# yuliakot/snark-verifier-axiom

Hardware: AMD Instinct MI355X
Metric: BN254 G1 MSM points/sec at 2^20 + KZG pairings/sec; 1/2/4/8 GPU (higher is better)
Workload: dtype u32 (254-bit Montgomery field: bucket chain 9x29-bit limbs, elsewhere 8x32-bit)

## Files before the change

### snark-verifier-axiom_amd/csrc/msm.hip

```cpp
#include <hip/hip_runtime.h>

#include <algorithm>
#include <chrono>
#include <cmath>
#include <cstdio>
#include <cstdlib>
#include <cstring>
#include <atomic>
#include <functional>
#include <string>
#include <thread>
#include <type_traits>
#include <vector>

#include "curve.hpp"
#include "curve29.hpp"
#include "glv.hpp"
#include "host_ec.hpp"
#include "msm.hpp"
#include "msm_batch.hpp"
#include "quad.hpp"
#include "runtime.hpp"

namespace sv {
// ... 144 lines not shown
    } else {
      f(w, bits, 0u);
      carry = 0;
    }
  }
}

__device__ __forceinline__ Fr scalar_in(const uint4 q0, const uint4 q1, int mont_in, uint32_t* __restrict__ err) {
  Fr s;
  s.v[0] = q0.x; s.v[1] = q0.y; s.v[2] = q0.z; s.v[3] = q0.w;
  s.v[4] = q1.x; s.v[5] = q1.y; s.v[6] = q1.z; s.v[7] = q1.w;
  if (err && !s.is_reduced()) atomicOr(err, 2u);
  return mont_in ? fe_from_mont(s) : s;
}
__device__ __forceinline__ Fr load_scalar(const Fr* __restrict__ scalars, uint32_t i, int mont_in,
                                          uint32_t* __restrict__ err) {
  const uint4* p = reinterpret_cast<const uint4*>(scalars + i);
  const uint4 q0 = p[0], q1 = p[1];
  Fr s;
  s.v[0] = q0.x; s.v[1] = q0.y; s.v[2] = q0.z; s.v[3] = q0.w;
  s.v[4] = q1.x; s.v[5] = q1.y; s.v[6] = q1.z; s.v[7] = q1.w;
  if (err && !s.is_reduced()) atomicOr(err, 2u);
  return mont_in ? fe_from_mont(s) : s;
}

template <int C, bool GLV>
struct Digits {
  static constexpr int NB = GLV ? 128 : 255;
  static constexpr int W = num_windows<C, NB>();
  static constexpr int EP = GLV ? 2 * W : W;
  uint32_t h[GLV ? 2 : 1][GLV ? 4 : 8];
  uint32_t sgn[GLV ? 2 : 1];
  __device__ __forceinline__ void load(const Fr* __restrict__ scalars, uint32_t i, int mont_in,
                                       uint32_t* __restrict__ err) {
    from(load_scalar(scalars, i, mont_in, err));
  }
  __device__ __forceinline__ void from(const Fr& s) {
    if constexpr (GLV) {
      uint32_t h1[4], h2[4];
      glv_split(s.v, h1, h2);
#pragma unroll
      for (int k = 0; k < 4; k++) h[0][k] = h1[k], h[1][k] = h2[k];
#pragma unroll
      for (int q = 0; q < 2; q++) {
        sgn[q] = h[q][3] >> 31;
        h[q][3] &= 0x7fffffffu;
      }
    } else {
#pragma unroll
      for (int k = 0; k < 8; k++) h[0][k] = s.v[k];
      sgn[0] = 0;
    }
  }
  __device__ __forceinline__ void store(uint4* __restrict__ hv, uint32_t i) const {
    if constexpr (GLV) {
      hv[2 * i] = make_uint4(h[0][0], h[0][1], h[0][2], h[0][3] | (sgn[0] << 31));
      hv[2 * i + 1] = make_uint4(h[1][0], h[1][1], h[1][2], h[1][3] | (sgn[1] << 31));
    } else {
      hv[2 * i] = make_uint4(h[0][0], h[0][1], h[0][2], h[0][3]);
      hv[2 * i + 1] = make_uint4(h[0][4], h[0][5], h[0][6], h[0][7]);
    }
  }
  __device__ __forceinline__ void load_stored(const uint4* __restrict__ hv, uint32_t i) {
    const uint4 a = hv[2 * i], b = hv[2 * i + 1];
    if constexpr (GLV) {
      h[0][0] = a.x; h[0][1] = a.y; h[0][2] = a.z; h[0][3] = a.w & 0x7fffffffu;
      h[1][0] = b.x; h[1][1] = b.y; h[1][2] = b.z; h[1][3] = b.w & 0x7fffffffu;
      sgn[0] = a.w >> 31;
      sgn[1] = b.w >> 31;
    } else {
      h[0][0] = a.x; h[0][1] = a.y; h[0][2] = a.z; h[0][3] = a.w;
      h[0][4] = b.x; h[0][5] = b.y; h[0][6] = b.z; h[0][7] = b.w;
      sgn[0] = 0;
    }
  }
  template <class F>
  __device__ __forceinline__ void each(F&& f) const {
#pragma unroll
    for (int q = 0; q < (GLV ? 2 : 1); q++) {
      Fr s;
      if constexpr (GLV) {
#pragma unroll
        for (int k = 0; k < 4; k++) s.v[k] = h[q][k], s.v[4 + k] = 0u;
      } else {
#pragma unroll
        for (int k = 0; k < 8; k++) s.v[k] = h[0][k];
      }
      const uint32_t sg = sgn[q];
      for_each_digit<C, NB>(s, [&](int w, uint32_t mag, uint32_t neg) { f(w, mag, neg ^ sg, (uint32_t)q); });
    }
  }
};

__device__ __forceinline__ void glv_phix(const G1Aff* __restrict__ bases, uint32_t i, uint4* __restrict__ phix,
                                         int phi64, uint32_t* __restrict__ err) {
  const uint4* b = reinterpret_cast<const uint4*>(bases + i);
  Fq x, beta;
  const uint4 x0 = b[0], x1 = b[1];
  x.v[0] = x0.x; x.v[1] = x0.y; x.v[2] = x0.z; x.v[3] = x0.w;
  x.v[4] = x1.x; x.v[5] = x1.y; x.v[6] = x1.z; x.v[7] = x1.w;
#pragma unroll
  for (int j = 0; j < 8; j++) beta.v[j] = GLV_BETA_MONT[j];
  const Fq bx = x * beta;
  uint4* o = phix + (phi64 ? 4 : 2) * i;
  o[0] = make_uint4(bx.v[0], bx.v[1], bx.v[2], bx.v[3]);
  o[1] = make_uint4(bx.v[4], bx.v[5], bx.v[6], bx.v[7]);
  if (phi64 || err) {
    const uint4 y0 = b[2], y1 = b[3];
    if (phi64) {
      o[2] = y0;
      o[3] = y1;
    }
    if (err) {
      Fq y;
      y.v[0] = y0.x; y.v[1] = y0.y; y.v[2] = y0.z; y.v[3] = y0.w;
      y.v[4] = y1.x; y.v[5] = y1.y; y.v[6] = y1.z; y.v[7] = y1.w;
      if (!x.is_reduced() || !y.is_reduced()) atomicOr(err, 1u);
    }
  }
}

__global__ void k_glv_phix(const G1Aff* __restrict__ bases, uint32_t n, uint4* __restrict__ phix, int phi64,
                           uint32_t* __restrict__ err) {
  const uint32_t i = blockIdx.x * blockDim.x + threadIdx.x;
  if (i < n) glv_phix(bases, i, phix, phi64, err);
}

static constexpr int kPhiVtab = 2;
static constexpr int kVtabRec = 9;
static constexpr uint32_t kVtabIdentity = 0x80000000u;
__device__ __forceinline__ void st_rec29(uint2* o, const r29::F& x, const r29::F& y) {
  o[0] = make_uint2(x.v[0], x.v[1]);
  o[1] = make_uint2(x.v[2], x.v[3]);
  o[2] = make_uint2(x.v[4], x.v[5]);
  o[3] = make_uint2(x.v[6], x.v[7]);
  o[4] = make_uint2(x.v[8], y.v[0]);
  o[5] = make_uint2(y.v[1], y.v[2]);
  o[6] = make_uint2(y.v[3], y.v[4]);
  o[7] = make_uint2(y.v[5], y.v[6]);
  o[8] = make_uint2(y.v[7], y.v[8]);
}
__device__ __forceinline__ void ld_rec29(const uint2* __restrict__ o, r29::F& x, r29::F& y) {
  uint2 q[kVtabRec];
#pragma unroll
  for (int k = 0; k < kVtabRec; k++) q[k] = o[k];
  x.v[0] = q[0].x, x.v[1] = q[0].y, x.v[2] = q[1].x, x.v[3] = q[1].y, x.v[4] = q[2].x, x.v[5] = q[2].y;
  x.v[6] = q[3].x, x.v[7] = q[3].y, x.v[8] = q[4].x;
  y.v[0] = q[4].y, y.v[1] = q[5].x, y.v[2] = q[5].y, y.v[3] = q[6].x, y.v[4] = q[6].y, y.v[5] = q[7].x;
  y.v[6] = q[7].y, y.v[7] = q[8].x, y.v[8] = q[8].y;
}
__device__ __forceinline__ void vtab_put_pt(const G1Aff& a, uint32_t i, uint4* __restrict__ vtab, uint32_t nsplit,
                                            bool glv, uint32_t* __restrict__ err) {
  if (err && (!a.x.is_reduced() || !a.y.is_reduced())) atomicOr(err, 1u);
  r29::F y = r29::to_r29(a.y.v);
  const r29::F x = r29::to_r29(a.x.v);
  if (r29::is_zero(x) && r29::is_zero(y)) y.v[r29::L - 1] = kVtabIdentity;
  uint2* t = reinterpret_cast<uint2*>(vtab);
  st_rec29(t + kVtabRec * (size_t)i, x, y);
  if (glv) {
    constexpr uint32_t kBeta29[r29::L] = {0xa337995u, 0x158d1d23u, 0x189c9b98u, 0x12fa4e45u, 0x185faadcu,
                                         0x176f16du, 0xeed93bau,  0x14291140u, 0xc0afeu};
    r29::F beta;
#pragma unroll
    for (int j = 0; j < r29::L; j++) beta.v[j] = kBeta29[j];
    st_rec29(t + kVtabRec * ((size_t)nsplit + i), r29::mul(x, beta), y);
  }
}
__device__ __forceinline__ void vtab_put(const G1Aff* __restrict__ bases, uint32_t i, uint4* __restrict__ vtab,
                                         uint32_t nsplit, bool glv, uint32_t* __restrict__ err) {
  vtab_put_pt(load_aff(bases, i), i, vtab, nsplit, glv, err);
}
__global__ void k_vtab(const G1Aff* __restrict__ bases, uint32_t n, uint4* __restrict__ vtab, int glv,
                       uint32_t* __restrict__ err) {
  const uint32_t i = blockIdx.x * blockDim.x + threadIdx.x;
  if (i < n) vtab_put(bases, i, vtab, n, glv != 0, err);
}

__global__ void __launch_bounds__(kBlock) k_resident_prepare(const G1Aff* in, G1Aff* out, uint32_t n, int mont_in,
                                                             uint4* __restrict__ vtab, uint32_t* __restrict__ err) {
  const uint32_t i = blockIdx.x * blockDim.x + threadIdx.x;
  if (i >= n) return;
  G1Aff a;
  {
    const uint4* p = reinterpret_cast<const uint4*>(in + i);
    const uint4 q0 = p[0], q1 = p[1], q2 = p[2], q3 = p[3];
    a.x.v[0] = q0.x; a.x.v[1] = q0.y; a.x.v[2] = q0.z; a.x.v[3] = q0.w;
    a.x.v[4] = q1.x; a.x.v[5] = q1.y; a.x.v[6] = q1.z; a.x.v[7] = q1.w;
    a.y.v[0] = q2.x; a.y.v[1] = q2.y; a.y.v[2] = q2.z; a.y.v[3] = q2.w;
    a.y.v[4] = q3.x; a.y.v[5] = q3.y; a.y.v[6] = q3.z; a.y.v[7] = q3.w;
  }
  if (!a.x.is_reduced() || !a.y.is_reduced()) {
    atomicOr(err, 1u);
    a.x = Fq::zero();
    a.y = Fq::zero();
  }
  if (!mont_in && !a.is_identity()) {
    a.x = fe_to_mont(a.x);
    a.y = fe_to_mont(a.y);
  }
  uint4* o = reinterpret_cast<uint4*>(out + i);
  o[0] = make_uint4(a.x.v[0], a.x.v[1], a.x.v[2], a.x.v[3]);
  o[1] = make_uint4(a.x.v[4], a.x.v[5], a.x.v[6], a.x.v[7]);
  o[2] = make_uint4(a.y.v[0], a.y.v[1], a.y.v[2], a.y.v[3]);
  o[3] = make_uint4(a.y.v[4], a.y.v[5], a.y.v[6], a.y.v[7]);
  vtab_put_pt(a, i, vtab, n, true, nullptr);
}

__global__ void k_check_bases(const G1Aff* __restrict__ bases, uint32_t n, uint32_t* __restrict__ err) {
  const uint32_t i = blockIdx.x * blockDim.x + threadIdx.x;
  if (i >= n) return;
  const G1Aff a = load_aff(bases, i);
  if (!a.x.is_reduced() || !a.y.is_reduced()) atomicOr(err, 1u);
}

__host__ __device__ constexpr int ceil_log2(int x) { return x <= 1 ? 0 : 1 + ceil_log2((x + 1) / 2); }

template <int N>
__device__ __forceinline__ uint32_t block_excl_scan(uint32_t* x, uint32_t* part) {
  constexpr int PER = (N + kBlock - 1) / kBlock;
  const int tid = threadIdx.x;
  uint32_t loc[PER];
  uint32_t sum = 0;
#pragma unroll
  for (int j = 0; j < PER; j++) {
    const int k = tid * PER + j;
    loc[j] = k < N ? x[k] : 0u;
    sum += loc[j];
  }
  part[tid] = sum;
  __syncthreads();
  for (int off = 1; off < kBlock; off <<= 1) {
    const uint32_t u = tid >= off ? part[tid - off] : 0u;
    __syncthreads();
    part[tid] += u;
    __syncthreads();
  }
  uint32_t run = part[tid] - sum;
  const uint32_t total = part[kBlock - 1];
#pragma unroll
  for (int j = 0; j < PER; j++) {
    const int k = tid * PER + j;
    if (k < N) x[k] = run;
    run += loc[j];
  }
  __syncthreads();
  return total;
}

__device__ __forceinline__ uint32_t pack_entry32(uint32_t fine, uint32_t neg, uint32_t pt, uint32_t fb) {
  return (fb ? fine << (32 - fb) : 0u) | (neg << (31 - fb)) | pt;
}
__device__ __forceinline__ uint64_t load_entry(const uint64_t* __restrict__ tmp, uint32_t i, int e32, uint32_t fb) {
  if (!e32) return tmp[i];
  const uint32_t v = reinterpret_cast<const uint32_t*>(tmp)[i];
  const uint32_t fine = fb ? v >> (32 - fb) : 0u, neg = (v >> (31 - fb)) & 1u, pt = v & ((1u << (31 - fb)) - 1u);
  return ((uint64_t)fine << 32) | pt | (neg << 31);
}

__device__ __forceinline__ uint32_t sort_block(uint32_t b, uint32_t n, int xcd) {
  const uint32_t nfull = n & ~7u;
  if (!xcd || b >= nfull) return b;
  return (b & 7u) * (nfull >> 3) + (b >> 3);
}

template <int C, bool GLV>
__global__ void __launch_bounds__(kBlock) k_bin_hist(const Fr* __restrict__ scalars, uint32_t n, int mont_in,
                                                     uint32_t nblk, uint32_t* __restrict__ bcnt,
                                                     uint32_t* __restrict__ err, const G1Aff* __restrict__ bases,
                                                     uint4* __restrict__ phix, int phi64, int check_bases,
                                                     int xcd, int bm, uint32_t w0, uint32_t nw,
                                                     uint4* __restrict__ stored, int pf) {
  using D = Digits<C, GLV>;
  constexpr int W = D::W, LOGB = C - 1;
  constexpr int CB = coarse_bits(C, D::NB), FB = LOGB - CB, NBIN = 1 << CB;
  const uint32_t nk = nw * NBIN;
  __shared__ uint32_t h[W * NBIN];
  for (int k = threadIdx.x; k < W * NBIN; k += kBlock) h[k] = 0;
  __syncthreads();
  constexpr uint32_t CH = sort_chunk(D::EP);
  const uint32_t blk = sort_block(blockIdx.x, gridDim.x, xcd);
  const uint32_t lo = blk * CH, hi = min(n, lo + CH);
  auto count = [&](const D& d) {
    d.each([&](int w, uint32_t mag, uint32_t, uint32_t) {
      if (mag && (uint32_t)w - w0 < nw) atomicAdd(&h[(w - w0) * NBIN + ((mag - 1) >> FB)], 1u);
    });
  };
  if (phix && phi64 == kPhiVtab && pf) {
    uint32_t i = lo + threadIdx.x;
    const uint4* sp = reinterpret_cast<const uint4*>(scalars);
    const uint4* bp = reinterpret_cast<const uint4*>(bases);
    uint4 s0{}, s1{}, b0{}, b1{}, b2{}, b3{};
    if (i < hi) {
      s0 = sp[2 * (size_t)i], s1 = sp[2 * (size_t)i + 1];
      b0 = bp[4 * (size_t)i], b1 = bp[4 * (size_t)i + 1], b2 = bp[4 * (size_t)i + 2], b3 = bp[4 * (size_t)i + 3];
    }
    for (; i < hi; i += kBlock) {
      G1Aff a;
      a.x.v[0] = b0.x; a.x.v[1] = b0.y; a.x.v[2] = b0.z; a.x.v[3] = b0.w;
      a.x.v[4] = b1.x; a.x.v[5] = b1.y; a.x.v[6] = b1.z; a.x.v[7] = b1.w;
      a.y.v[0] = b2.x; a.y.v[1] = b2.y; a.y.v[2] = b2.z; a.y.v[3] = b2.w;
      a.y.v[4] = b3.x; a.y.v[5] = b3.y; a.y.v[6] = b3.z; a.y.v[7] = b3.w;
      const uint4 c0 = s0, c1 = s1;
      const uint32_t j = i + kBlock;
      if (j < hi) {
        s0 = sp[2 * (size_t)j], s1 = sp[2 * (size_t)j + 1];
        b0 = bp[4 * (size_t)j], b1 = bp[4 * (size_t)j + 1], b2 = bp[4 * (size_t)j + 2], b3 = bp[4 * (size_t)j + 3];
      }
      vtab_put_pt(a, i, phix, n, GLV, check_bases ? err : nullptr);
      D d;
      d.from(scalar_in(c0, c1, mont_in, err));
      if (stored) d.store(stored, i);
      count(d);
    }
  } else
  for (uint32_t i = lo + threadIdx.x; i < hi; i += kBlock) {
    if (phix && phi64 == kPhiVtab) {
      vtab_put(bases, i, phix, n, GLV, check_bases ? err : nullptr);
    } else if constexpr (GLV) {
      if (phix) glv_phix(bases, i, phix, phi64, check_bases ? err : nullptr);
    } else {
      if (check_bases) {
        const G1Aff a = load_aff(bases, i);
        if (!a.x.is_reduced() || !a.y.is_reduced()) atomicOr(err, 1u);
      }
    }
    D d;
    d.load(scalars, i, mont_in, err);
    if (stored) d.store(stored, i);
    count(d);
  }
  __syncthreads();
  for (uint32_t k = threadIdx.x; k < nk; k += kBlock)
    bcnt[bm ? (size_t)blk * nk + k : (size_t)k * nblk + blk] = h[k];
}

__global__ void __launch_bounds__(kBlock) k_bin_scan_chunks(uint32_t* __restrict__ bcnt, uint32_t nblk,
                                                            uint32_t* __restrict__ btot) {
  __shared__ uint32_t part[kBlock];
  uint32_t* c = bcnt + (size_t)blockIdx.x * nblk;
  const uint32_t tid = threadIdx.x, per = (nblk + kBlock - 1) / kBlock;
// ... 1001 lines not shown
  int device;
  size_t n;
  int mont_in;
  const MsmFeed* feed;
  const MsmResident* res;
  MsmTuning t;
  MsmPlan p;
  MsmShape s;
  bool lean, detail;
  uint32_t r_off, r_phi;
  const uint4* r_tab;
  const G1Aff* bases;
  const Fr* scalars;
  G1Aff* bases_m;
  uint4 *phix, *stored;
  G1Xyzz *ping, *bsum, *racc, *rtot, *gpart, *tree_out;
  uint32_t *gst_all, *ent_all, *tst_all;
  MsmScratch w;
  std::vector<SortOut> so;
  const uint32_t* half_gst[2] = {nullptr, nullptr};

  hipEvent_t ev(int slot) const { return ws->ev[slot]; }
  hipEvent_t ev_if(bool on, int slot) const { return on ? ws->ev[slot] : nullptr; }
};

struct SortArgs {
  const G1Aff* bases = nullptr;
  const Fr* scalars = nullptr;
  size_t m = 0;
  uint4* phix = nullptr;
  uint32_t nsplit = ~0u, p_off = 0;
  int check_bases = 0;
  uint32_t w0 = 0, nw = 0;
  uint4* stored = nullptr;
  hipStream_t st = nullptr;
  hipStream_t side = nullptr;
  hipEvent_t ev_mid = nullptr, ev_fork = nullptr, ev_join = nullptr;
};
static int msm_sort(const MsmCall& c, const SortOut& so, const SortArgs& a) {
  const MsmPlan& p = c.p;
  const MsmTuning& t = c.t;
  const MsmScratch& w = c.w;
  hipStream_t st = a.st;
  const int LOGB = p.c - 1;
  const int nb = p.glv ? 128 : 255;
  const uint32_t CB = (uint32_t)coarse_bits(p.c, nb), FB = (uint32_t)LOGB - CB, NBIN = 1u << CB;
  const uint32_t w0 = a.w0, nw = a.nw ? a.nw : p.W;
  const uint32_t nwb = nw * NBIN;
  const uint32_t npts = (uint32_t)a.m;
  const uint32_t ep = p.glv ? 2 * p.W : p.W;
  const uint32_t nblk = cdiv(npts, sort_chunk((int)ep));
  const uint64_t vmax = p.glv ? (uint64_t)a.nsplit + npts : (uint64_t)a.p_off + npts;
  const int e32 = vmax <= (uint64_t(1) << (31 - FB)) && t.sort_e32 ? 1 : 0;
  const int xcd = t.sort_xcd, bm = t.sort_bm, hist_pf = t.hist_pf;
  const int mont_in = c.mont_in;
  SV_LAUNCH_C(k_bin_hist, p.glv, p.c, dim3(nblk), dim3(kBlock), a.scalars, npts, mont_in, nblk, w.bcnt, w.err,
              a.bases, a.phix, p.r29 ? kPhiVtab : p.phi64, a.check_bases, xcd, bm, w0, nw, a.stored, hist_pf);
  SV_HIP(hipGetLastError());
  if (a.ev_mid) SV_HIP(hipEventRecord(a.ev_mid, st));
  if (bm) {
    if (t.scan_keys == 16)
      hipLaunchKernelGGL(k_bin_scan_tiles<16>, dim3(cdiv(nwb, 16)), dim3(1024), 0, st, w.bcnt, nblk, nwb, w.btot);
    else
      hipLaunchKernelGGL(k_bin_scan_tiles<32>, dim3(cdiv(nwb, 32)), dim3(1024), 0, st, w.bcnt, nblk, nwb, w.btot);
  } else {
    hipLaunchKernelGGL(k_bin_scan_chunks, dim3(nwb), dim3(kBlock), 0, st, w.bcnt, nblk, w.btot);
  }
  hipLaunchKernelGGL(k_bin_scan, dim3(1), dim3(1024), 0, st, w.btot, nwb, w.bstart, so.gst + (size_t)nw * p.B);
  SV_LAUNCH_C(k_bin_scatter, p.glv, p.c, dim3(nblk), dim3(kBlock), a.scalars, npts, mont_in, nblk, w.bcnt, w.btot,
              w.bstart, w.tmp, e32, xcd, bm, w0, nw, a.stored, a.p_off, p.glv ? a.nsplit : 0u);
  static thread_local int fine_attr_dev = -1;
  if (fine_attr_dev != c.device) {
    SV_HIP(hipFuncSetAttribute(reinterpret_cast<const void*>(&k_fine_sort<0>),
                               hipFuncAttributeMaxDynamicSharedMemorySize, (int)kFineLds));
    SV_HIP(hipFuncSetAttribute(reinterpret_cast<const void*>(&k_fine_sort<1>),
                               hipFuncAttributeMaxDynamicSharedMemorySize, (int)kFineLds));
    SV_HIP(hipFuncSetAttribute(reinterpret_cast<const void*>(&k_fine_sort<2>),
                               hipFuncAttributeMaxDynamicSharedMemorySize, (int)kFineLds));
    fine_attr_dev = c.device;
  }
  if (!t.fine_split && !a.side) {
    hipLaunchKernelGGL(k_fine_sort<2>, dim3(nwb), dim3(1024), kFineLds, st, w.tmp, e32, w.bstart, FB, so.K, so.gst,
                       so.tstart, so.ent);
    SV_HIP(hipGetLastError());
    return SV_OK;
  }
  hipStream_t big_st = a.side ? a.side : st;
  if (a.side) {
    SV_HIP(hipEventRecord(a.ev_fork, st));
    SV_HIP(hipStreamWaitEvent(a.side, a.ev_fork, 0));
  }
  hipLaunchKernelGGL(k_fine_sort<1>, dim3(nwb), dim3(1024), kFineLds, big_st, w.tmp, e32, w.bstart, FB, so.K,
                     so.gst, so.tstart, so.ent);
  hipLaunchKernelGGL(k_fine_sort<0>, dim3(nwb), dim3(1024), kFineLds, st, w.tmp, e32, w.bstart, FB, so.K, so.gst,
                     so.tstart, so.ent);
  if (a.side) {
    SV_HIP(hipEventRecord(a.ev_join, a.side));
    SV_HIP(hipStreamWaitEvent(st, a.ev_join, 0));
  }
  SV_HIP(hipGetLastError());
  return SV_OK;
}

struct AccArgs {
  const G1Aff* bases = nullptr;
  const uint4* phix = nullptr;
  uint32_t nsplit = ~0u;
  int add_into = 0;
  G1Xyzz* bsum = nullptr;
  uint32_t nbt = 0;
// ... 223 lines not shown
    const std::vector<size_t>& pb = c_.s.pb;
    hipStream_t cs = c_.ws->copy_stream;
    int rc = SV_OK;
    try {
      int st0;
      while ((st0 = staged_.load(std::memory_order_acquire)) == 0 && !stop_.load(std::memory_order_relaxed))
        std::this_thread::yield();
      for (int k = 0; st0 > 0 && k < c_.s.pieces && !stop_.load(std::memory_order_relaxed); k++) {
        const size_t lo = pb[k], hi = pb[k + 1];
        if (k > 0) {
          rc = feed->stage_scalars(lo, hi, const_cast<Fr*>(c_.scalars) + lo, cs, c_.ev(ev_slot::piece_scalars(k)));
          if (rc != SV_OK) break;
          staged_.store(scalars_of(k), std::memory_order_release);
        }
        if (!c_.res)
          rc = feed->stage_bases(lo, hi, const_cast<G1Aff*>(c_.bases) + lo, cs, c_.ev(ev_slot::piece_bases(k)));
        if (rc != SV_OK) break;
        staged_.store(bases_of(k), std::memory_order_release);
      }
    } catch (const std::exception& e) {
      set_error("host-fed MSM feeder: %s", e.what());
      rc = SV_ERR_DEVICE;
    } catch (...) {
      set_error("host-fed MSM feeder: unknown exception");
      rc = SV_ERR_DEVICE;
    }
    if (rc != SV_OK) fail(rc);
  }

  const MsmCall& c_;
  std::atomic<int> staged_{0}, stop_{0};
  int rc_ = SV_OK;
  std::string err_;
  bool started_ = false;
};

static int prepare_piece(const MsmCall& c, Feeder& feeder, int k, uint4* phix_k, const G1Aff** pbases) {
  const MsmPlan& p = c.p;
  const size_t lo = c.s.pb[k], m = c.s.pb[k + 1] - lo;
  hipStream_t st = c.ws->stream, ss = c.ws->sort_stream;
  hipEvent_t sorted = c.ev(ev_slot::piece_sorted(k));
  const bool conv = c.s.conv;
  G1Aff* db = const_cast<G1Aff*>(c.bases) + lo;
  if (!c.t.fed_prep) SV_HIP(hipEventRecord(sorted, ss));
  SV_TRY(feeder.wait(Feeder::bases_of(k)));
  hipStream_t ps = c.t.fed_prep ? ss : st;
  SV_HIP(hipStreamWaitEvent(ps, c.ev(ev_slot::piece_bases(k)), 0));
  *pbases = conv ? c.bases_m + lo : db;
  if (conv)
    hipLaunchKernelGGL(k_to_mont_bases, dim3(cdiv(m, kBlock)), dim3(kBlock), 0, ps, db, c.bases_m + lo, (uint32_t)m,
                       c.w.err);
  if (p.r29)
    hipLaunchKernelGGL(k_vtab, dim3(cdiv(m, kBlock)), dim3(kBlock), 0, ps, *pbases, (uint32_t)m, phix_k,
                       p.glv ? 1 : 0, conv ? nullptr : c.w.err);
  else if (!p.glv)
    hipLaunchKernelGGL(k_check_bases, dim3(cdiv(m, kBlock)), dim3(kBlock), 0, ps, db, (uint32_t)m, c.w.err);
  if (!p.r29 && p.glv)
    hipLaunchKernelGGL(k_glv_phix, dim3(cdiv(m, kBlock)), dim3(kBlock), 0, ps, *pbases, (uint32_t)m, phix_k, p.phi64,
                       conv ? nullptr : c.w.err);
  SV_HIP(hipGetLastError());
  if (c.t.fed_prep) SV_HIP(hipEventRecord(sorted, ss));
  return SV_OK;
}

static int run_fed(MsmCall& c) {
  namespace ev = ev_slot;
  const MsmPlan& p = c.p;
  const MsmShape& s = c.s;
  Workspace* ws = c.ws;
  hipStream_t st = ws->stream, cs = ws->copy_stream, ss = ws->sort_stream;
  const bool res = c.res != nullptr;
  if (s.pieces > 1) SV_HIP(hipMemsetAsync(c.bsum, 0, (size_t)p.nbt * s.rec_bytes, st));
  SV_HIP(hipEventRecord(c.ev(ev::kFedFork), st));
  SV_HIP(hipStreamWaitEvent(cs, c.ev(ev::kFedFork), 0));
  SV_HIP(hipStreamWaitEvent(ss, c.ev(ev::kFedFork), 0));
  Feeder feeder(c);
  SV_TRY(feeder.start());
  for (int k = 0; k < s.pieces; k++) {
    const size_t lo = s.pb[k], m = s.pb[k + 1] - lo;
    const uint32_t lo32 = (uint32_t)lo;
    hipEvent_t sorted = c.ev(ev::piece_sorted(k));
    const uint32_t nsplit = p.glv ? (res ? c.r_phi + lo32 : (uint32_t)m) : ~0u;
    uint4* phix_k = s.tab4 ? c.phix + s.tab4 * lo : nullptr;
    SV_TRY(feeder.wait(Feeder::scalars_of(k)));
    SV_HIP(hipStreamWaitEvent(ss, c.ev(ev::piece_scalars(k)), 0));
    SV_TRY(msm_sort(c, c.so[k], {.scalars = c.scalars + lo, .m = m, .nsplit = nsplit,
                                 .p_off = res ? c.r_off + lo32 : 0u, .st = ss}));
    const G1Aff* pbases = nullptr;
    if (res) SV_HIP(hipEventRecord(sorted, ss));
    else SV_TRY(prepare_piece(c, feeder, k, phix_k, &pbases));
    SV_HIP(hipStreamWaitEvent(st, sorted, 0));
    if (k == 0) SV_HIP(hipEventRecord(c.ev(ev::kAccBegin), st));
    SV_TRY(msm_acc(c, scratch_of(c, k), c.so[k],
                   {.bases = pbases, .phix = res ? c.r_tab : phix_k, .nsplit = res ? ~0u : nsplit,
                    .add_into = k > 0 ? 1 : 0, .bsum = c.bsum, .st = st,
                    .ev_acc_done = c.ev_if(k == s.pieces - 1, ev::kAccEnd)}));
  }
  return SV_OK;
}

static int reduce_buckets(const MsmCall& c) {
  const MsmPlan& p = c.p;
  const MsmShape& s = c.s;
  hipStream_t st = c.ws->stream;
  const uint32_t* gst = s.pieces > 1 ? nullptr : c.so[0].gst;
  if (p.tree == 0) {
    hipLaunchKernelGGL(k_wsum, dim3(cdiv((uint64_t)p.J * p.W, kBlock)), dim3(kBlock), 0, st, c.bsum, gst, p.B, p.J,
// ... 122 lines not shown
  c.t = msm_tuning();
  if (n <= kSmallMsmTerms && c.t.small_msm) return run_small(c.ws, d_bases, d_scalars, n, form, device, feed, res, out);
  c.device = device;
  c.n = n;
  c.mont_in = form == SV_MONTGOMERY ? 1 : 0;
  c.feed = feed;
  c.res = res;
  c.p = msm_plan(n, c.t);
  if (res) c.p.r29 = 1;
  MsmMode mode;
  mode.canonical = form == SV_CANONICAL;
  mode.fed = feed != nullptr;
  mode.resident = res != nullptr;
  if (feed) mode.pieces = feed->pieces, mode.split = feed->split;
  c.s = msm_shape(n, mode, c.p, c.t);
  c.lean = c.t.msm_lean;
  c.detail = c.t.msm_stats && !c.lean;
  c.r_off = res ? (uint32_t)res->off : 0u;
  c.r_phi = res ? (uint32_t)(res->N + res->off) : 0u;
  c.r_tab = res ? reinterpret_cast<const uint4*>(res->vtab) : nullptr;
  SV_TRY(lay_out(c, mode, d_bases, d_scalars));

  hipStream_t st = c.ws->stream;
  Drain drain{c.ws, feed != nullptr || c.s.split};
  if (!c.lean) SV_HIP(hipEventRecord(c.ev(ev_slot::kStart), st));
  SV_HIP(hipMemsetAsync(c.w.err, 0, c.s.nerr * 4, st));
  SV_TRY(feed ? run_fed(c) : c.s.split ? run_device_split(c) : run_device(c));
  SV_TRY(reduce_buckets(c));
  if (!c.lean) SV_HIP(hipEventRecord(c.ev(ev_slot::kEnd), st));
  return finish(c, drain, out);
}

int msm_run_device(const void* d_bases, const void* d_scalars, size_t n, int form, int device,
                   hipStream_t user_stream, host::Xyzz* out) {
  return msm_run_impl(d_bases, d_scalars, n, form, device, user_stream, nullptr, out);
}

int msm_run_fed(size_t n, int form, int device, const MsmFeed& feed, host::Xyzz* out) {
  return msm_run_impl(nullptr, nullptr, n, form, device, nullptr, &feed, out);
}

int msm_resident_prepare(const void* d_rows, size_t n, int form, int device, hipStream_t user_stream,
                         void* d_rows_m, void* d_vtab) {
  WsLease lease(device, user_stream);
  if (!lease.ok()) return SV_ERR_DEVICE;
  Workspace* ws = lease.get();
  hipStream_t st = ws->stream;
  SV_TRY(ws->reserve(256));
  SV_TRY(ws->reserve_pinned(256));
  uint32_t* err = ws->carve<uint32_t>(1);
  SV_HIP(hipMemsetAsync(err, 0, 4, st));
  hipLaunchKernelGGL(k_resident_prepare, dim3(cdiv(n, kBlock)), dim3(kBlock), 0, st,
                     reinterpret_cast<const G1Aff*>(d_rows), reinterpret_cast<G1Aff*>(d_rows_m), (uint32_t)n,
                     form == SV_MONTGOMERY ? 1 : 0, reinterpret_cast<uint4*>(d_vtab), err);
  SV_HIP(hipGetLastError());
  SV_HIP(hipMemcpyAsync(ws->pinned, err, 4, hipMemcpyDeviceToHost, st));
  SV_HIP(hipStreamSynchronize(st));
  uint32_t errv;
  memcpy(&errv, ws->pinned, 4);
  if (errv) {
    set_error("invalid input: base coordinate not reduced mod p");
    return SV_ERR_ARG;
  }
  return SV_OK;
}

int msm_run_resident_device(const MsmResident& set, const void* d_scalars, size_t n, int form, int device,
                            hipStream_t user_stream, host::Xyzz* out) {
  return msm_run_impl(nullptr, d_scalars, n, form, device, user_stream, nullptr, out, &set);
}

int msm_run_resident_fed(const MsmResident& set, size_t n, int form, int device, const MsmFeed& feed,
                         host::Xyzz* out) {
  return msm_run_impl(nullptr, nullptr, n, form, device, nullptr, &feed, out, &set);
}

}
```

### snark-verifier-axiom_amd/csrc/msm_plan.hpp

```cpp
#pragma once
#include <algorithm>
#include <cstddef>
#include <cstdint>
#include <cstdlib>
#include <vector>

#include "field29.hpp"

#if defined(__HIPCC__) || defined(__HIP__)
#define SV_PLAN_HD __host__ __device__
#define SV_PLAN_HDI __host__ __device__ __forceinline__
#else
#define SV_PLAN_HD
#define SV_PLAN_HDI inline
#endif

namespace sv {

constexpr int kBlock = 256;

constexpr size_t kSmallMsmTerms = 256;

constexpr size_t kFrBytes = 32, kAffBytes = 64, kXyzzBytes = 128;

constexpr uint32_t kRec29Words = 4 * r29::L;
SV_PLAN_HDI size_t bucket_rec_bytes(int r29) { return r29 ? 4 * kRec29Words : kXyzzBytes; }

SV_PLAN_HD constexpr size_t vtab_uint4_per_point(bool glv) { return glv ? 9 : 5; }

#ifndef SV_SORT_CHUNK
#define SV_SORT_CHUNK 1024
#endif
SV_PLAN_HD constexpr uint32_t sort_chunk(int ep) {
  return ep > 20 ? 256u : (ep > 16 && SV_SORT_CHUNK > 1024 ? 1024u : (uint32_t)SV_SORT_CHUNK);
}
SV_PLAN_HD constexpr int coarse_bits(int c, int nb) { return c - 1 < (nb == 128 ? 7 : 6) ? c - 1 : (nb == 128 ? 7 : 6); }

constexpr int kTreeLog = 8, kTreeN = 1 << kTreeLog;
constexpr int kTreeOut = 2 + kTreeLog;

inline uint32_t cdiv(uint64_t a, uint64_t b) { return (uint32_t)((a + b - 1) / b); }

struct MsmTuning {
  struct Opt {
    bool set = false;
    int v = 0;
  };
  Opt acc_k;
  Opt glv;
  int glv_max_log = 21;
  Opt glv_phi64;
  Opt window_bits;
  Opt red_log;
  int group_tree = 1;
  bool group_quad = true;
  Opt group_p;
  bool acc_r29 = true;
  bool sort_e32 = true;
  bool sort_xcd = true;
  bool sort_bm = true;
  bool hist_pf = true;
  int scan_keys = 32;
  bool fine_split = false;
  bool sort_fork = false;
  bool sort_halves = true;
  bool msm_split = false;
  bool msm_stats = false;
  bool msm_lean = false;
  bool fed_prep = true;
  bool small_msm = true;
  std::vector<double> h2d_split;
};

inline MsmTuning msm_tuning() {
  auto opt = [](const char* name) {
    MsmTuning::Opt o;
    if (const char* e = getenv(name)) o.set = true, o.v = atoi(e);
    return o;
  };
  auto on = [](const char* name) { return !getenv(name) || atoi(getenv(name)) != 0; };
  auto off = [](const char* name) { return getenv(name) && atoi(getenv(name)) != 0; };
  MsmTuning t;
  t.acc_k = opt("SVGPU_ACC_K");
  t.glv = opt("SVGPU_GLV");
  if (const char* e = getenv("SVGPU_GLV_MAX_LOG")) t.glv_max_log = atoi(e);
  t.glv_phi64 = opt("SVGPU_GLV_PHI64");
  t.window_bits = opt("SVGPU_WINDOW_BITS");
  t.red_log = opt("SVGPU_RED_LOG");
  if (const char* e = getenv("SVGPU_GROUP_TREE")) t.group_tree = atoi(e);
  t.group_quad = on("SVGPU_GROUP_QUAD");
  t.group_p = opt("SVGPU_GROUP_P");
  t.acc_r29 = on("SVGPU_ACC_R29");
  t.sort_e32 = on("SVGPU_SORT_E32");
  static const bool xcd = on("SVGPU_SORT_XCD"), bm = on("SVGPU_SORT_BM"), stats = off("SVGPU_MSM_STATS");
  t.sort_xcd = xcd;
  t.sort_bm = bm;
  t.msm_stats = stats;
  t.hist_pf = on("SVGPU_HIST_PF");
  if (const char* e = getenv("SVGPU_SCAN_KEYS")) t.scan_keys = atoi(e) == 16 ? 16 : 32;
  t.fine_split = off("SVGPU_FINE_SPLIT");
  t.sort_fork = off("SVGPU_SORT_FORK");
  t.sort_halves = on("SVGPU_SORT_HALVES");
  t.msm_split = off("SVGPU_MSM_SPLIT");
  t.msm_lean = off("SVGPU_MSM_LEAN");
  t.fed_prep = on("SVGPU_FED_PREP");
  t.small_msm = on("SVGPU_SMALL_MSM");
  if (const char* e = getenv("SVGPU_H2D_SPLIT")) {
    for (const char* q = e; *q;) {
      char* end = nullptr;
      const double v = strtod(q, &end);
      if (end == q) break;
      if (v > 0) t.h2d_split.push_back(v);
      q = *end == ',' ? end + 1 : end;
      if (*end && *end != ',') break;
    }
  }
  return t;
}

struct MsmPlan {
  int c;
  uint32_t W;
  uint32_t B;
  uint32_t nbt;
  uint32_t K;
  uint32_t T;
  uint32_t logL;
  uint32_t J;
  uint32_t logJ;
  uint32_t NG;
  bool glv;
  size_t npts;
  int phi64;
  int tree;
  int r29;
};

inline uint32_t plan_K(uint64_t entries, uint32_t nbt, const MsmTuning& t) {
  uint64_t K = entries / (1u << 18);
  if (K < 4) K = 4;
  if (K > 32) K = 32;
  const uint64_t avg_bucket = entries / nbt;
  if (K < avg_bucket) K = avg_bucket < 256 ? avg_bucket : 256;
  if (t.acc_k.set) K = (uint64_t)t.acc_k.v;
  if (K < 1) K = 1;
  return (uint32_t)K;
}

inline uint32_t piece_K(uint64_t entries, uint32_t nbt, const MsmTuning& t) {
  if (t.acc_k.set) return plan_K(entries, nbt, t);
  const uint64_t avg = entries / nbt;
// ... 231 lines not shown
```

Measured before the change: 674.6 million.

## Stage vtab and scalar-digit stores through per-wave LDS tiles for coalesced writes

Vtab records of 9 uint2 per point and the stored GLV digit halves are now written into a per-wave LDS tile first and then flushed so consecutive lanes write consecutive words, instead of each lane writing its own strided record. This applies to k_vtab, k_resident_prepare and the fused histogram/prep path in k_bin_hist. The goal is to turn strided global stores into coalesced ones, at the cost of extra LDS traffic, wave-level barriers and more shared memory per block. A SVGPU_HIST_TILE knob (default 1) selects the new path.

```diff
diff --git a/snark-verifier-axiom_amd/csrc/msm.hip b/snark-verifier-axiom_amd/csrc/msm.hip
--- a/snark-verifier-axiom_amd/csrc/msm.hip
+++ b/snark-verifier-axiom_amd/csrc/msm.hip
@@ -220,14 +220,20 @@
       sgn[0] = 0;
     }
   }
+  __device__ __forceinline__ void halves(uint4& a, uint4& b) const {
+    if constexpr (GLV) {
+      a = make_uint4(h[0][0], h[0][1], h[0][2], h[0][3] | (sgn[0] << 31));
+      b = make_uint4(h[1][0], h[1][1], h[1][2], h[1][3] | (sgn[1] << 31));
+    } else {
+      a = make_uint4(h[0][0], h[0][1], h[0][2], h[0][3]);
+      b = make_uint4(h[0][4], h[0][5], h[0][6], h[0][7]);
+    }
+  }
   __device__ __forceinline__ void store(uint4* __restrict__ hv, uint32_t i) const {
-    if constexpr (GLV) {
-      hv[2 * i] = make_uint4(h[0][0], h[0][1], h[0][2], h[0][3] | (sgn[0] << 31));
-      hv[2 * i + 1] = make_uint4(h[1][0], h[1][1], h[1][2], h[1][3] | (sgn[1] << 31));
-    } else {
-      hv[2 * i] = make_uint4(h[0][0], h[0][1], h[0][2], h[0][3]);
-      hv[2 * i + 1] = make_uint4(h[0][4], h[0][5], h[0][6], h[0][7]);
-    }
+    uint4 a, b;
+    halves(a, b);
+    hv[2 * i] = a;
+    hv[2 * i + 1] = b;
   }
   __device__ __forceinline__ void load_stored(const uint4* __restrict__ hv, uint32_t i) {
     const uint4 a = hv[2 * i], b = hv[2 * i + 1];
@@ -295,7 +301,7 @@
 }
 
 static constexpr int kPhiVtab = 2;
-static constexpr int kVtabRec = 9;
+static constexpr int kVtabRec = kVtabRecU2;
 static constexpr uint32_t kVtabIdentity = 0x80000000u;
 __device__ __forceinline__ void st_rec29(uint2* o, const r29::F& x, const r29::F& y) {
   o[0] = make_uint2(x.v[0], x.v[1]);
@@ -317,61 +323,121 @@
   y.v[0] = q[4].y, y.v[1] = q[5].x, y.v[2] = q[5].y, y.v[3] = q[6].x, y.v[4] = q[6].y, y.v[5] = q[7].x;
   y.v[6] = q[7].y, y.v[7] = q[8].x, y.v[8] = q[8].y;
 }
+__device__ __forceinline__ void vtab_limbs(const G1Aff& a, uint32_t* __restrict__ err, r29::F& x, r29::F& y) {
+  if (err && (!a.x.is_reduced() || !a.y.is_reduced())) atomicOr(err, 1u);
+  y = r29::to_r29(a.y.v);
+  x = r29::to_r29(a.x.v);
+  if (r29::is_zero(x) && r29::is_zero(y)) y.v[r29::L - 1] = kVtabIdentity;
+}
+__device__ __forceinline__ r29::F vtab_beta_x(const r29::F& x) {
+  constexpr uint32_t kBeta29[r29::L] = {0xa337995u, 0x158d1d23u, 0x189c9b98u, 0x12fa4e45u, 0x185faadcu,
+                                       0x176f16du, 0xeed93bau,  0x14291140u, 0xc0afeu};
+  r29::F beta;
+#pragma unroll
+  for (int j = 0; j < r29::L; j++) beta.v[j] = kBeta29[j];
+  return r29::mul(x, beta);
+}
 __device__ __forceinline__ void vtab_put_pt(const G1Aff& a, uint32_t i, uint4* __restrict__ vtab, uint32_t nsplit,
                                             bool glv, uint32_t* __restrict__ err) {
-  if (err && (!a.x.is_reduced() || !a.y.is_reduced())) atomicOr(err, 1u);
-  r29::F y = r29::to_r29(a.y.v);
-  const r29::F x = r29::to_r29(a.x.v);
-  if (r29::is_zero(x) && r29::is_zero(y)) y.v[r29::L - 1] = kVtabIdentity;
+  r29::F x, y;
+  vtab_limbs(a, err, x, y);
   uint2* t = reinterpret_cast<uint2*>(vtab);
   st_rec29(t + kVtabRec * (size_t)i, x, y);
-  if (glv) {
-    constexpr uint32_t kBeta29[r29::L] = {0xa337995u, 0x158d1d23u, 0x189c9b98u, 0x12fa4e45u, 0x185faadcu,
-                                         0x176f16du, 0xeed93bau,  0x14291140u, 0xc0afeu};
-    r29::F beta;
-#pragma unroll
-    for (int j = 0; j < r29::L; j++) beta.v[j] = kBeta29[j];
-    st_rec29(t + kVtabRec * ((size_t)nsplit + i), r29::mul(x, beta), y);
-  }
+  if (glv) st_rec29(t + kVtabRec * ((size_t)nsplit + i), vtab_beta_x(x), y);
 }
 __device__ __forceinline__ void vtab_put(const G1Aff* __restrict__ bases, uint32_t i, uint4* __restrict__ vtab,
                                          uint32_t nsplit, bool glv, uint32_t* __restrict__ err) {
   vtab_put_pt(load_aff(bases, i), i, vtab, nsplit, glv, err);
 }
-__global__ void k_vtab(const G1Aff* __restrict__ bases, uint32_t n, uint4* __restrict__ vtab, int glv,
-                       uint32_t* __restrict__ err) {
+
+__device__ __forceinline__ void wave_lds_sync() {
+  __builtin_amdgcn_fence(__ATOMIC_RELEASE, "wavefront");
+  __builtin_amdgcn_wave_barrier();
+  __builtin_amdgcn_fence(__ATOMIC_ACQUIRE, "wavefront");
+}
+constexpr uint32_t kVtabTileWords = 2 * kVtabTileU2;
+__device__ __forceinline__ void vtab_tile_flush(const uint32_t* tile, uint32_t lane, uint32_t cnt,
+                                                uint2* __restrict__ dst) {
+  const uint2* t2 = reinterpret_cast<const uint2*>(tile);
+#pragma unroll
+  for (uint32_t k = 0; k < kVtabRecU2; k++)
+    if (vtab_tile_live(k, lane, cnt)) dst[vtab_tile_word(k, lane)] = t2[vtab_tile_word(k, lane)];
+}
+__device__ __forceinline__ void vtab_tile_store(uint32_t* tile, uint32_t lane, uint32_t cnt, const r29::F& x,
+                                                const r29::F& y, uint4* __restrict__ vtab, size_t rec0,
+                                                size_t nsplit, bool glv) {
+  uint2* t = reinterpret_cast<uint2*>(vtab);
+  uint2* mine = reinterpret_cast<uint2*>(tile) + vtab_tile_slot(lane, 0);
+  st_rec29(mine, x, y);
+  wave_lds_sync();
+  vtab_tile_flush(tile, lane, cnt, t + vtab_rec_u2(rec0));
+  if (glv) {
+    const r29::F bx = vtab_beta_x(x);
+    wave_lds_sync();
+    mine[0] = make_uint2(bx.v[0], bx.v[1]);
+    mine[1] = make_uint2(bx.v[2], bx.v[3]);
+    mine[2] = make_uint2(bx.v[4], bx.v[5]);
+    mine[3] = make_uint2(bx.v[6], bx.v[7]);
+    tile[2 * vtab_tile_slot(lane, 4)] = bx.v[8];
+    wave_lds_sync();
+    vtab_tile_flush(tile, lane, cnt, t + vtab_rec_u2(nsplit + rec0));
+  }
+  wave_lds_sync();
+}
+__device__ __forceinline__ uint32_t wave_in_block() { return __builtin_amdgcn_readfirstlane(threadIdx.x >> 6); }
+
+__global__ void __launch_bounds__(kBlock) k_vtab(const G1Aff* __restrict__ bases, uint32_t n,
+                                                 uint4* __restrict__ vtab, int glv, uint32_t* __restrict__ err,
+                                                 int tile) {
   const uint32_t i = blockIdx.x * blockDim.x + threadIdx.x;
-  if (i < n) vtab_put(bases, i, vtab, n, glv != 0, err);
+  if (!tile) {
+    if (i < n) vtab_put(bases, i, vtab, n, glv != 0, err);
+    return;
+  }
+  __shared__ __align__(16) uint32_t tiles[kBlock / kWaveLanes][kVtabTileWords];
+  const uint32_t wv = wave_in_block(), i0 = blockIdx.x * kBlock + kWaveLanes * wv;
+  if (i0 >= n) return;
+  r29::F x{}, y{};
+  if (i < n) vtab_limbs(load_aff(bases, i), err, x, y);
+  vtab_tile_store(tiles[wv], threadIdx.x & 63u, min(kWaveLanes, n - i0), x, y, vtab, i0, n, glv != 0);
 }
 
 __global__ void __launch_bounds__(kBlock) k_resident_prepare(const G1Aff* in, G1Aff* out, uint32_t n, int mont_in,
-                                                             uint4* __restrict__ vtab, uint32_t* __restrict__ err) {
+                                                             uint4* __restrict__ vtab, uint32_t* __restrict__ err,
+                                                             int tile) {
+  __shared__ __align__(16) uint32_t tiles[kBlock / kWaveLanes][kVtabTileWords];
   const uint32_t i = blockIdx.x * blockDim.x + threadIdx.x;
-  if (i >= n) return;
+  const uint32_t wv = wave_in_block(), i0 = blockIdx.x * kBlock + kWaveLanes * wv;
+  if (i0 >= n) return;
+  const bool live = i < n;
   G1Aff a;
-  {
+  if (live) {
     const uint4* p = reinterpret_cast<const uint4*>(in + i);
     const uint4 q0 = p[0], q1 = p[1], q2 = p[2], q3 = p[3];
     a.x.v[0] = q0.x; a.x.v[1] = q0.y; a.x.v[2] = q0.z; a.x.v[3] = q0.w;
     a.x.v[4] = q1.x; a.x.v[5] = q1.y; a.x.v[6] = q1.z; a.x.v[7] = q1.w;
     a.y.v[0] = q2.x; a.y.v[1] = q2.y; a.y.v[2] = q2.z; a.y.v[3] = q2.w;
     a.y.v[4] = q3.x; a.y.v[5] = q3.y; a.y.v[6] = q3.z; a.y.v[7] = q3.w;
-  }
-  if (!a.x.is_reduced() || !a.y.is_reduced()) {
-    atomicOr(err, 1u);
-    a.x = Fq::zero();
-    a.y = Fq::zero();
-  }
-  if (!mont_in && !a.is_identity()) {
-    a.x = fe_to_mont(a.x);
-    a.y = fe_to_mont(a.y);
-  }
-  uint4* o = reinterpret_cast<uint4*>(out + i);
-  o[0] = make_uint4(a.x.v[0], a.x.v[1], a.x.v[2], a.x.v[3]);
-  o[1] = make_uint4(a.x.v[4], a.x.v[5], a.x.v[6], a.x.v[7]);
-  o[2] = make_uint4(a.y.v[0], a.y.v[1], a.y.v[2], a.y.v[3]);
-  o[3] = make_uint4(a.y.v[4], a.y.v[5], a.y.v[6], a.y.v[7]);
-  vtab_put_pt(a, i, vtab, n, true, nullptr);
+    if (!a.x.is_reduced() || !a.y.is_reduced()) {
+      atomicOr(err, 1u);
+      a.x = Fq::zero();
+      a.y = Fq::zero();
+    }
+    if (!mont_in && !a.is_identity()) {
+      a.x = fe_to_mont(a.x);
+      a.y = fe_to_mont(a.y);
+    }
+    uint4* o = reinterpret_cast<uint4*>(out + i);
+    o[0] = make_uint4(a.x.v[0], a.x.v[1], a.x.v[2], a.x.v[3]);
+    o[1] = make_uint4(a.x.v[4], a.x.v[5], a.x.v[6], a.x.v[7]);
+    o[2] = make_uint4(a.y.v[0], a.y.v[1], a.y.v[2], a.y.v[3]);
+    o[3] = make_uint4(a.y.v[4], a.y.v[5], a.y.v[6], a.y.v[7]);
+    if (!tile) vtab_put_pt(a, i, vtab, n, true, nullptr);
+  }
+  if (!tile) return;
+  r29::F x{}, y{};
+  if (live) vtab_limbs(a, nullptr, x, y);
+  vtab_tile_store(tiles[wv], threadIdx.x & 63u, min(kWaveLanes, n - i0), x, y, vtab, i0, n, true);
 }
 
 __global__ void k_check_bases(const G1Aff* __restrict__ bases, uint32_t n, uint32_t* __restrict__ err) {
@@ -437,7 +503,7 @@
                                                      uint32_t* __restrict__ err, const G1Aff* __restrict__ bases,
                                                      uint4* __restrict__ phix, int phi64, int check_bases,
                                                      int xcd, int bm, uint32_t w0, uint32_t nw,
-                                                     uint4* __restrict__ stored, int pf) {
+                                                     uint4* __restrict__ stored, int pf, int tile) {
   using D = Digits<C, GLV>;
   constexpr int W = D::W, LOGB = C - 1;
   constexpr int CB = coarse_bits(C, D::NB), FB = LOGB - CB, NBIN = 1 << CB;
@@ -453,7 +519,52 @@
       if (mag && (uint32_t)w - w0 < nw) atomicAdd(&h[(w - w0) * NBIN + ((mag - 1) >> FB)], 1u);
     });
   };
-  if (phix && phi64 == kPhiVtab && pf) {
+  if (phix && phi64 == kPhiVtab && tile) {
+    __shared__ __align__(16) uint32_t tiles[kBlock / kWaveLanes][kVtabTileWords];
+    const uint32_t lane = threadIdx.x & 63u, wv = wave_in_block();
+    uint32_t* tl = tiles[wv];
+    const uint4* sp = reinterpret_cast<const uint4*>(scalars);
+    const uint4* bp = reinterpret_cast<const uint4*>(bases);
+    uint4 s0{}, s1{}, b0{}, b1{}, b2{}, b3{};
+    auto fetch = [&](uint32_t j) {
+      if (j < hi) {
+        s0 = sp[2 * (size_t)j], s1 = sp[2 * (size_t)j + 1];
+        b0 = bp[4 * (size_t)j], b1 = bp[4 * (size_t)j + 1], b2 = bp[4 * (size_t)j + 2], b3 = bp[4 * (size_t)j + 3];
+      }
+    };
+    uint32_t i0 = lo + kWaveLanes * wv;
+    if (pf) fetch(i0 + lane);
+    for (; i0 < hi; i0 += kBlock) {
+      const uint32_t i = i0 + lane, cnt = min(kWaveLanes, hi - i0);
+      const bool live = i < hi;
+      if (!pf) fetch(i);
+      G1Aff a;
+      a.x.v[0] = b0.x; a.x.v[1] = b0.y; a.x.v[2] = b0.z; a.x.v[3] = b0.w;
+      a.x.v[4] = b1.x; a.x.v[5] = b1.y; a.x.v[6] = b1.z; a.x.v[7] = b1.w;
+      a.y.v[0] = b2.x; a.y.v[1] = b2.y; a.y.v[2] = b2.z; a.y.v[3] = b2.w;
+      a.y.v[4] = b3.x; a.y.v[5] = b3.y; a.y.v[6] = b3.z; a.y.v[7] = b3.w;
+      const uint4 c0 = s0, c1 = s1;
+      if (pf) fetch(i + kBlock);
+      r29::F x{}, y{};
+      if (live) vtab_limbs(a, check_bases ? err : nullptr, x, y);
+      vtab_tile_store(tl, lane, cnt, x, y, phix, i0, n, GLV);
+      D d{};
+      if (live) d.from(scalar_in(c0, c1, mont_in, err));
+      if (stored && tile == 1) {
+        uint4* t4 = reinterpret_cast<uint4*>(tl);
+        d.halves(t4[2 * lane], t4[2 * lane + 1]);
+        wave_lds_sync();
+        uint4* hv = stored + 2 * (size_t)i0;
+#pragma unroll
+        for (uint32_t k = 0; k < 2; k++)
+          if (kWaveLanes * k + lane < 2 * cnt) hv[kWaveLanes * k + lane] = t4[kWaveLanes * k + lane];
+        wave_lds_sync();
+      } else if (stored && live) {
+        d.store(stored, i);
+      }
+      if (live) count(d);
+    }
+  } else if (phix && phi64 == kPhiVtab && pf) {
     uint32_t i = lo + threadIdx.x;
     const uint4* sp = reinterpret_cast<const uint4*>(scalars);
     const uint4* bp = reinterpret_cast<const uint4*>(bases);
@@ -1561,10 +1672,10 @@
   const uint32_t nblk = cdiv(npts, sort_chunk((int)ep));
   const uint64_t vmax = p.glv ? (uint64_t)a.nsplit + npts : (uint64_t)a.p_off + npts;
   const int e32 = vmax <= (uint64_t(1) << (31 - FB)) && t.sort_e32 ? 1 : 0;
-  const int xcd = t.sort_xcd, bm = t.sort_bm, hist_pf = t.hist_pf;
+  const int xcd = t.sort_xcd, bm = t.sort_bm, hist_pf = t.hist_pf, hist_tile = t.hist_tile;
   const int mont_in = c.mont_in;
   SV_LAUNCH_C(k_bin_hist, p.glv, p.c, dim3(nblk), dim3(kBlock), a.scalars, npts, mont_in, nblk, w.bcnt, w.err,
-              a.bases, a.phix, p.r29 ? kPhiVtab : p.phi64, a.check_bases, xcd, bm, w0, nw, a.stored, hist_pf);
+              a.bases, a.phix, p.r29 ? kPhiVtab : p.phi64, a.check_bases, xcd, bm, w0, nw, a.stored, hist_pf, hist_tile);
   SV_HIP(hipGetLastError());
   if (a.ev_mid) SV_HIP(hipEventRecord(a.ev_mid, st));
   if (bm) {
@@ -1894,7 +2005,7 @@
                        c.w.err);
   if (p.r29)
     hipLaunchKernelGGL(k_vtab, dim3(cdiv(m, kBlock)), dim3(kBlock), 0, ps, *pbases, (uint32_t)m, phix_k,
-                       p.glv ? 1 : 0, conv ? nullptr : c.w.err);
+                       p.glv ? 1 : 0, conv ? nullptr : c.w.err, c.t.hist_tile);
   else if (!p.glv)
     hipLaunchKernelGGL(k_check_bases, dim3(cdiv(m, kBlock)), dim3(kBlock), 0, ps, db, (uint32_t)m, c.w.err);
   if (!p.r29 && p.glv)
@@ -2123,7 +2234,7 @@
   SV_HIP(hipMemsetAsync(err, 0, 4, st));
   hipLaunchKernelGGL(k_resident_prepare, dim3(cdiv(n, kBlock)), dim3(kBlock), 0, st,
                      reinterpret_cast<const G1Aff*>(d_rows), reinterpret_cast<G1Aff*>(d_rows_m), (uint32_t)n,
-                     form == SV_MONTGOMERY ? 1 : 0, reinterpret_cast<uint4*>(d_vtab), err);
+                     form == SV_MONTGOMERY ? 1 : 0, reinterpret_cast<uint4*>(d_vtab), err, msm_tuning().hist_tile);
   SV_HIP(hipGetLastError());
   SV_HIP(hipMemcpyAsync(ws->pinned, err, 4, hipMemcpyDeviceToHost, st));
   SV_HIP(hipStreamSynchronize(st));
diff --git a/snark-verifier-axiom_amd/csrc/msm_plan.hpp b/snark-verifier-axiom_amd/csrc/msm_plan.hpp
--- a/snark-verifier-axiom_amd/csrc/msm_plan.hpp
+++ b/snark-verifier-axiom_amd/csrc/msm_plan.hpp
@@ -27,6 +27,16 @@
 SV_PLAN_HDI size_t bucket_rec_bytes(int r29) { return r29 ? 4 * kRec29Words : kXyzzBytes; }
 
 SV_PLAN_HD constexpr size_t vtab_uint4_per_point(bool glv) { return glv ? 9 : 5; }
+
+constexpr uint32_t kWaveLanes = 64;
+constexpr uint32_t kVtabRecU2 = 9;
+constexpr uint32_t kVtabTileU2 = kVtabRecU2 * kWaveLanes;
+SV_PLAN_HD constexpr uint32_t vtab_tile_slot(uint32_t lane, uint32_t j) { return kVtabRecU2 * lane + j; }
+SV_PLAN_HD constexpr uint32_t vtab_tile_word(uint32_t k, uint32_t lane) { return kWaveLanes * k + lane; }
+SV_PLAN_HD constexpr bool vtab_tile_live(uint32_t k, uint32_t lane, uint32_t cnt) {
+  return vtab_tile_word(k, lane) < kVtabRecU2 * cnt;
+}
+SV_PLAN_HD constexpr size_t vtab_rec_u2(size_t rec) { return (size_t)kVtabRecU2 * rec; }
 
 #ifndef SV_SORT_CHUNK
 #define SV_SORT_CHUNK 1024
@@ -60,6 +70,7 @@
   bool sort_xcd = true;
   bool sort_bm = true;
   bool hist_pf = true;
+  int hist_tile = 1;
   int scan_keys = 32;
   bool fine_split = false;
   bool sort_fork = false;
@@ -97,6 +108,7 @@
   t.sort_bm = bm;
   t.msm_stats = stats;
   t.hist_pf = on("SVGPU_HIST_PF");
+  if (const char* e = getenv("SVGPU_HIST_TILE")) t.hist_tile = atoi(e) == 2 ? 2 : atoi(e) != 0;
   if (const char* e = getenv("SVGPU_SCAN_KEYS")) t.scan_keys = atoi(e) == 16 ? 16 : 32;
   t.fine_split = off("SVGPU_FINE_SPLIT");
   t.sort_fork = off("SVGPU_SORT_FORK");
```

After: 681.3 million (median of 6 runs). About the same (+1.0%).
